# 7IBBE77S/nbodysim

Measured on AMD Instinct MI355X. Metric: particle-pair interactions/sec at N=262,144 (direct O(N^2) softened gravity + kick/drift step), higher is better.
Workload: dtype f32

## Files before the change

### include/nbody.h

```cpp
#ifndef NBODY_H
#define NBODY_H

#include <stddef.h>
#include <stdint.h>

#ifdef __cplusplus
extern "C" {
#endif
#pragma GCC visibility push(default)

#define NB_ABI_VERSION 8

typedef struct nb_vec2 {
    float x, y;
    float _pad[2];
} nb_vec2;

#define NB_Z(v) ((v)._pad[0])

typedef struct nb_body {
    nb_vec2 pos;
    nb_vec2 vel;
    nb_vec2 acc;
    float   mass;
// ... 69 lines not shown
       NB_INTEGRATOR_KDK = 1 };

enum { NB_FLAG_NO_SYMMETRY     = 1,
       NB_FLAG_NO_UNIFORM_MASS = 2,
       NB_FLAG_NO_GUIDED_TAIL  = 4,
       NB_FLAG_SHARD_ALLREDUCE = 8,
       NB_FLAG_MASS_SCALING    = 32,
       NB_FLAG_MASS_SCALING_MEASURED = 1024,
       NB_FLAG_NO_MASS_SCALING = 512,
       NB_FLAG_STATIC_ITEMS    = 256,
       NB_FLAG_SHARD_SINGLE    = 16,
       NB_FLAG_TREE_LEAVES     = 4096,
       NB_FLAG_TREE_QUADRUPOLE = 8192,
       NB_FLAG_TREE_ENERGY = 16384,
       NB_FLAG_TREE_RELATIVE = 32768 };
enum { NB_FLAGS_KNOWN = NB_FLAG_NO_SYMMETRY | NB_FLAG_NO_UNIFORM_MASS | NB_FLAG_NO_GUIDED_TAIL | NB_FLAG_SHARD_ALLREDUCE | NB_FLAG_SHARD_SINGLE |
                        NB_FLAG_MASS_SCALING | NB_FLAG_NO_MASS_SCALING | NB_FLAG_STATIC_ITEMS | NB_FLAG_MASS_SCALING_MEASURED |
                        NB_FLAG_TREE_LEAVES | NB_FLAG_TREE_QUADRUPOLE | NB_FLAG_TREE_ENERGY | NB_FLAG_TREE_RELATIVE };

typedef struct nb_params {
    uint32_t struct_size;
    float    eps;
    float    dt;
    int32_t  precision;
    int32_t  rsqrt_mode;
    int32_t  sum_order;
    int32_t  integrator;
    int32_t  extras;
    int32_t  device;
    int32_t  j_slices;
    uint64_t i_begin;
    uint64_t i_count;
    void    *stream;
// ... 63 lines not shown
    uint32_t struct_size;
    uint32_t width, height;
    float    center_x, center_y, scale;
    float    mass_quantum;
    uint32_t _reserved0;
} nb_view;
int nb_raster(nb_sim *s, const nb_view *view, uint32_t *count, float *mass);

#define NB_NO_NEIGHBOR 0xFFFFFFFFu
int nb_neighbors(nb_sim *s, float radius, uint32_t k, uint32_t *idx, float *dist2, uint32_t *count);

int nb_groups(nb_sim *s, float radius, uint32_t *label, uint32_t *size, uint64_t *ngroups);

int nb_tree_alpha(nb_sim *s, float alpha);

uint64_t nb_frame(const nb_sim *s);
size_t   nb_count(const nb_sim *s);
size_t   nb_owned_begin(const nb_sim *s);
size_t   nb_owned_count(const nb_sim *s);

int nb_dump(nb_sim *s, const char *path);
int nb_write_bodies(const char *path, const nb_body *bodies, size_t n, uint64_t frame,
                    const nb_params *params);
int nb_read_header(const char *path, size_t *n, uint64_t *frame, nb_params *params);
int nb_read_bodies(const char *path, nb_body *out, size_t n);

enum { NB_POS_CURRENT = 0, NB_POS_NEXT = 1 };
enum { NB_SHARD_NONE = 0, NB_SHARD_ALLGATHER = 1, NB_SHARD_SYMMETRIC = 2, NB_SHARD_ALLREDUCE = 3 };
int   nb_shard_protocol(const nb_sim *s);
int   nb_exchange_positions(nb_sim *const *sims, int count);
// ... 74 lines not shown
```

### nbodysim_amd/_lib.py

```python
from __future__ import annotations

import ctypes as C
import os
from pathlib import Path

import numpy as np

PKG_DIR = Path(__file__).resolve().parent
LIB_PATH = PKG_DIR / "libnbody_hip.so"

NB_ABI_VERSION = 8

NB_OK, NB_EINVAL, NB_ENODEVICE, NB_EHIP, NB_ENOMEM, NB_EIO, NB_EFORMAT, NB_ESTATE = 0, -1, -2, -3, -4, -5, -6, -7
NB_FP32, NB_FP64 = 0, 1
NB_RSQRT_EXACT, NB_RSQRT_QUAKE = 0, 1
NB_SUM_TILED, NB_SUM_SEQUENTIAL = 0, 1
NB_EXTRA_VCLAMP, NB_EXTRA_BOUNDARY, NB_EXTRA_COLLIDE = 1, 2, 4
NB_INTEGRATOR_KICK_DRIFT, NB_INTEGRATOR_KDK = 0, 1
NB_FORCE_DIRECT, NB_FORCE_TREE = 0, 1
NB_POS_CURRENT, NB_POS_NEXT = 0, 1
NB_SHARD_NONE, NB_SHARD_ALLGATHER, NB_SHARD_SYMMETRIC, NB_SHARD_ALLREDUCE = 0, 1, 2, 3
NB_FLAG_NO_SYMMETRY, NB_FLAG_NO_UNIFORM_MASS, NB_FLAG_NO_GUIDED_TAIL, NB_FLAG_SHARD_ALLREDUCE, NB_FLAG_SHARD_SINGLE, NB_FLAG_MASS_SCALING = 1, 2, 4, 8, 16, 32
NB_FLAG_STATIC_ITEMS = 256
NB_FLAG_NO_MASS_SCALING = 512
NB_FLAG_MASS_SCALING_MEASURED = 1024
NB_FLAG_TREE_LEAVES = 4096
NB_FLAG_TREE_QUADRUPOLE = 8192
NB_FLAG_TREE_ENERGY = 16384
NB_FLAG_TREE_RELATIVE = 32768
NB_NO_NEIGHBOR = 0xFFFFFFFF

BODY_DTYPE = np.dtype(
    {
        "names": ["pos", "vel", "acc", "mass", "radius"],
        "formats": [(np.float32, 2), (np.float32, 2), (np.float32, 2), np.float32, np.float32],
        "offsets": [0, 16, 32, 48, 52],
        "itemsize": 64,
    }
)


BODY3_DTYPE = np.dtype(
    {
        "names": ["pos", "vel", "acc", "mass", "radius"],
# ... 131 lines not shown
    "nb_snapshot_wait": (C.c_int, [C.c_void_p]),
    "nb_host_register": (C.c_int, [C.c_void_p, C.c_size_t]),
    "nb_host_unregister": (C.c_int, [C.c_void_p]),
    "nb_host_alloc": (C.c_void_p, [C.c_size_t]),
    "nb_host_free": (C.c_int, [C.c_void_p]),
    "nb_upload": (C.c_int, [C.c_void_p, C.c_void_p]),
    "nb_accelerations": (C.c_int, [C.c_void_p]),
    "nb_energy": (C.c_int, [C.c_void_p, C.POINTER(C.c_double), C.POINTER(C.c_double)]),
    "nb_momentum": (C.c_int, [C.c_void_p, C.POINTER(C.c_double), C.POINTER(C.c_double)]),
    "nb_potentials": (C.c_int, [C.c_void_p, C.c_void_p]),
    "nb_collide_capacity": (C.c_int, [C.c_void_p, C.c_size_t]),
    "nb_collision_stats": (C.c_int, [C.c_void_p, C.POINTER(C.c_uint64), C.POINTER(C.c_uint64), C.POINTER(C.c_uint32), C.POINTER(C.c_uint64)]),
    "nb_tree_stats": (C.c_int, [C.c_void_p, C.POINTER(C.c_uint64), C.POINTER(C.c_uint32), C.POINTER(C.c_uint64)]),
    "nb_tree_nodes": (C.c_int, [C.c_void_p, C.c_void_p, C.c_size_t, C.POINTER(C.c_size_t)]),
    "nb_tree_alpha": (C.c_int, [C.c_void_p, C.c_float]),
    "nb_raster": (C.c_int, [C.c_void_p, C.POINTER(nb_view), C.c_void_p, C.c_void_p]),
    "nb_neighbors": (C.c_int, [C.c_void_p, C.c_float, C.c_uint32, C.c_void_p, C.c_void_p, C.c_void_p]),
    "nb_groups": (C.c_int, [C.c_void_p, C.c_float, C.c_void_p, C.c_void_p, C.POINTER(C.c_uint64)]),
    "nb_frame": (C.c_uint64, [C.c_void_p]),
    "nb_count": (C.c_size_t, [C.c_void_p]),
    "nb_owned_begin": (C.c_size_t, [C.c_void_p]),
    "nb_owned_count": (C.c_size_t, [C.c_void_p]),
    "nb_dump": (C.c_int, [C.c_void_p, C.c_char_p]),
    "nb_write_bodies": (C.c_int, [C.c_char_p, C.c_void_p, C.c_size_t, C.c_uint64, C.POINTER(nb_params)]),
    "nb_read_header": (C.c_int, [C.c_char_p, C.POINTER(C.c_size_t), C.POINTER(C.c_uint64), C.POINTER(nb_params)]),
    "nb_read_bodies": (C.c_int, [C.c_char_p, C.c_void_p, C.c_size_t]),
    "nb_step_begin": (C.c_int, [C.c_void_p, C.c_float]),
    "nb_step_mid": (C.c_int, [C.c_void_p]),
    "nb_step_finish": (C.c_int, [C.c_void_p]),
    "nb_pos_buffer": (C.c_void_p, [C.c_void_p, C.c_int]),
# ... 129 lines not shown
```

### nbodysim_amd/csrc/nb_capi.hip

```cpp
#include "nb_sim.hip.h"

extern "C" int nb_device_count(void)
{
    int n = 0;
    if (hipGetDeviceCount(&n) != hipSuccess) { (void)hipGetLastError(); return 0; }
    return n;
}

static uint32_t even_slices(uint32_t jn, uint32_t want)
{
    const uint32_t tiles = (jn + TJ - 1) / TJ;
    if (want < 1) want = 1;
    if (want > tiles) want = tiles;
    const uint32_t per = (tiles + want - 1) / want;
    return (tiles + per - 1) / per;
}

static ForceJob plan_job(const nb_sim *s, uint32_t jb, uint32_t je, uint32_t slab0,
                         uint32_t gap_begin = 0xffffffffu, uint32_t gap_len = 0)
{
    ForceJob j{jb, je, 0, slab0, 1, 0, gap_begin, gap_len};
    const uint32_t ic = (uint32_t)s->i_count;
    if (je <= jb) return j;
    const uint32_t jn = je - jb;
// ... 28 lines not shown
    s->slabs_all = s->path == StepPath::SYM ? 1 : s->job_all.js;
    s->job_local = plan_job(s, ib, ib + ic, 0);
    s->job_remote = plan_job(s, 0, n - ic, s->job_local.js, ib, ic);
    s->slabs_two_phase = s->job_local.js + s->job_remote.js;
}

static bool needs_guard(const nb_sim *s) { return s->fp64 ? !(s->p.eps > 0.0f) : !(s->p.eps >= 1e-12f); }

static uint32_t sym_tile_of(const nb_params &p, size_t n)
{
    if (p.precision == NB_FP64 || p.dims == 3 || p.shard_world > 1 || (p.flags & NB_FLAG_SHARD_SINGLE)) return SYM_SB;
    if (p.sym_tile) return (uint32_t)p.sym_tile;
    return n < SYM_WS_MAX_N ? SYM_SB_WS : SYM_SB;
}

static bool sym_eligible(const nb_sim *s)
{
    if (s->p.flags & NB_FLAG_NO_SYMMETRY) return false;
    if (s->p.sum_order != NB_SUM_TILED || needs_guard(s)) return false;
    if (s->fp64 && s->p.rsqrt_mode != NB_RSQRT_EXACT) return false;
    if (s->p.integrator != NB_INTEGRATOR_KICK_DRIFT && s->i_count != s->n) return false;
    if (s->n < (sym_tile_of(s->p, s->n) == SYM_SB_WS ? (size_t)5632 : 8 * (size_t)SYM_SB)) return false;
    const uint32_t world = s->p.shard_world > 1 ? (uint32_t)s->p.shard_world : 1u;
    size_t cap = (size_t)96 << 30;
    if (world == 1) {
        size_t free_b = 0, total_b = 0;
        if (hipMemGetInfo(&free_b, &total_b) != hipSuccess) { (void)hipGetLastError(); free_b = (size_t)24 << 30; }
        if (free_b / 3 < cap) cap = free_b / 3;
    }
    if (sym_slab_r_bound((uint32_t)s->n, world, sym_tile_of(s->p, s->n)) * s->esz > cap) return false;
    return true;
}

static bool single_rank(const nb_sim *s)
{
    return (s->p.flags & NB_FLAG_SHARD_SINGLE) && s->p.shard_world == 1 && s->p.shard_rank == 0 && s->i_count == s->n;
}
// ... 352 lines not shown

static int query_stage(nb_sim *s, size_t bytes)
{
    HIPCHK(s->pool.regrow_pinned(s->qstage_cap, bytes, s->qstage));
    return NB_OK;
}

static int copy_plane(nb_sim *s, void *dst, const void *src, size_t bytes) { return copy_d2h(s, dst, src, bytes, s->stream, s->qstage); }

#include "nb_collide_host.hip.h"
#include "nb_tree_host.hip.h"
#include "nb_raster_host.hip.h"
#include "nb_potential_host.hip.h"
#include "nb_neighbors_host.hip.h"
#include "nb_groups_host.hip.h"

static int step_check(nb_sim *s)
{
    const int rc = collide_check(s);
    return rc ? rc : tree_check(s);
}

static int do_upload(nb_sim *s, const nb_body *in)
{
    { const int rc = fence_foreign_work(s); if (rc) return rc; }
    s->uniform_mass = s->n > 0 && !s->tree && !(s->p.flags & NB_FLAG_NO_UNIFORM_MASS) && s->p.sum_order == NB_SUM_TILED;
    for (size_t i = 1; s->uniform_mass && i < s->n; ++i)
        if (memcmp(&in[i].mass, &in[0].mass, sizeof(float)) != 0) s->uniform_mass = false;
    s->um_mass = in[0].mass;
    s->mass_scaled = false;
// ... 20 lines not shown
    const uint32_t n = (uint32_t)s->n, g = (n + BLOCK - 1) / BLOCK, ib = (uint32_t)s->i_begin, ic = (uint32_t)s->i_count;
    with_layout(s, [&](auto L) {
        using real = typename decltype(L)::real;
        using vec = typename decltype(L)::vec;
        for (int b = 0; b < 2; ++b)
            unpack_bodies<decltype(L)><<<g, BLOCK, 0, s->stream>>>(s->aos_dev, n, (vec *)s->pos[b], (real *)s->mass, (vec *)s->vel, (vec *)s->acc,
                                                                   s->radius, ib, ic);
    });
    HIPCHK(hipGetLastError());
    if (forced_scaling || auto_scaling) {
        if (!s->sigma) HIPCHK(s->pool.alloc(s->sigma, s->n));
        mass_sigma<<<g, BLOCK, 0, s->stream>>>((const float *)s->mass, s->sigma, n);
        HIPCHK(hipGetLastError());
    }
    s->mass_scaled = forced_scaling;
    if (s->collide) { const int rc = collide_classify(s, in); if (rc) return rc; }
    HIPCHK(hipStreamSynchronize(s->stream));
    s->acc_valid = false;
    if (auto_scaling) { const int rc = choose_mass_scaling(s); if (rc) return rc; }
    if (auto_scaling || was_uniform != s->uniform_mass || was_scaled != s->mass_scaled) s->sym_first_wave = 0;
    s->sym_first_wave_uniform = s->uniform_mass;
    s->sym_first_wave_scaled = s->mass_scaled;
    return NB_OK;
}

extern "C" nb_sim *nb_create(const nb_body *init, size_t n, const nb_params *params)
{
    nb_clear_error();
    nb_params p;
    if (params) {
// ... 131 lines not shown
    s->bh.theta2 = p.theta * p.theta;
    s->bh.leaves = s->tree && (p.flags & NB_FLAG_TREE_LEAVES) != 0;
    s->bh.quad = s->bh.leaves && (p.flags & NB_FLAG_TREE_QUADRUPOLE) != 0;
    s->bh.energy = s->bh.leaves && (p.flags & NB_FLAG_TREE_ENERGY) != 0;
    s->bh.rel = s->bh.leaves && (p.flags & NB_FLAG_TREE_RELATIVE) != 0;
    if ((e = s->pool.alloc(s->mass, n * s->rsz)) != hipSuccess) return fail("allocating mass", e);
    if ((e = s->pool.alloc(s->radius, n)) != hipSuccess) return fail("allocating radius", e);
    if ((e = s->pool.alloc(s->vel, s->i_count * r2)) != hipSuccess) return fail("allocating vel", e);
    if ((e = s->pool.alloc(s->acc, s->i_count * r2)) != hipSuccess) return fail("allocating acc", e);
    if ((e = s->pool.alloc(s->partial, s->tree ? r2 : (size_t)s->slabs_cap * s->i_count * r2)) != hipSuccess) return fail("allocating partial", e);
    if ((e = s->pool.alloc(s->aos_dev, n)) != hipSuccess) return fail("allocating aos", e);
    s->ered_blocks = (s->i_count + BLOCK - 1) / BLOCK;
    if ((e = s->pool.alloc(s->ered_dev, (s->bh.energy ? 4 : 2) * s->ered_blocks)) != hipSuccess) return fail("allocating energy", e);

    s->collide = (p.extras & NB_EXTRA_COLLIDE) != 0;
    if ((symmetric(s) && plan_sym(s) != NB_OK) || (s->collide && collide_alloc(s) != NB_OK) || (s->tree && tree_alloc(s) != NB_OK) ||
        do_upload(s, init) != NB_OK) { free_all(s); (void)hipGetLastError(); return nullptr; }
    return s;
}

extern "C" void nb_destroy(nb_sim *s) { free_all(s); }

extern "C" int nb_upload(nb_sim *s, const nb_body *in)
{
    if (!s || !in) return nb_fail(NB_EINVAL, "nb_upload: NULL argument");
    if (bind(s)) return NB_EHIP;
    if (snapshot_wait(s)) return nb_last_error_code();
    return do_upload(s, in);
}

static int prof_begin(nb_sim *s, std::pair<hipEvent_t, hipEvent_t> *pr, hipStream_t st)
{
// ... 60 lines not shown

static int launch_sym_items(nb_sim *s, uint32_t first, uint32_t count, hipStream_t st = nullptr)
{
    if (count == 0) return NB_OK;
    if (!st) st = s->stream;
    std::pair<hipEvent_t, hipEvent_t> pr;
    if (s->prof && prof_begin(s, &pr, st)) return NB_EHIP;
    const uint32_t n = (uint32_t)s->n;
    const SymItem *items = s->sym_items_dev + first;
    const uint32_t slot = first == 0 ? 0u : (first == s->sym_items_local ? 1u : 2u);
    const bool quake = s->p.rsqrt_mode == NB_RSQRT_QUAKE, um = s->uniform_mass, pairs = sym_uses_pairs(s);
    const int rc = with_layout(s, [&](auto L) -> int {
        using real = typename decltype(L)::real;
        using vec = typename decltype(L)::vec;
        const real eps2 = (real)s->p.eps * (real)s->p.eps, umv = um ? (real)s->um_mass : (real)1;
        const vec *pos = (const vec *)s->pos[s->cur];
        vec *ss = (vec *)s->sym_slab_s, *sr = (vec *)s->sym_slab_r;
        auto go = [&](auto kernel, auto... lead) { return launch_sym_kernel(s, kernel, count, slot, st, lead..., items, ss, sr, n, eps2, umv); };
        if constexpr (L.dims3 && std::is_same_v<real, double>)
            return with_flags([&](auto u) { return go(force_sym3_f64<u>, pos); }, um);
        else if constexpr (L.dims3)
            return with_flags([&](auto q, auto u, auto pp) { return go(force_sym3_f32<q ? RSQ_QUAKE : RSQ_EXACT, u, pp>, pos); }, quake, um, pairs);
        else if constexpr (std::is_same_v<real, double>)
            return with_flags([&](auto u) { return go(force_sym_f64<u>, pos, (const double *)s->mass); }, um);
        else
            return with_flags([&](auto q, auto pp, auto ws) {
                constexpr int RQ = q ? RSQ_QUAKE : RSQ_EXACT;
                const float *mass = (const float *)s->mass;
                if (um) return go(force_sym_f32<RQ, MM_UNIFORM, pp, ws>, pos, mass, s->sigma);
                if constexpr (RQ == RSQ_EXACT && !pp)
                    if (s->mass_scaled) return go(force_sym_f32<RSQ_EXACT, MM_SCALED, false, ws>, pos, mass, s->sigma);
                return go(force_sym_f32<RQ, MM_GENERAL, pp, ws>, pos, mass, s->sigma);
            }, quake, pairs, s->sym_sb == SYM_SB_WS);
    });
    if (rc) return rc;
    if (s->prof && prof_end(s, pr, st)) return NB_EHIP;
    return NB_OK;
}

static int launch_gather(nb_sim *s, bool fuse, const uint32_t *lo, const uint32_t *hi, const uint32_t *cb, const SymCov *cov,
                         uint32_t first, uint32_t cnt, void *dst, const void *add, double dt)
{
    const uint32_t n = (uint32_t)s->n, per = s->dims3 ? (uint32_t)GATHER_T : (uint32_t)GATHER_P, gg = (cnt + per - 1) / per;
    const int extras = fuse ? s->p.extras : 0, kd = fuse ? INTEG_KICK | INTEG_DRIFT : 0;
    with_layout(s, [&](auto L) {
        using real = typename decltype(L)::real;
        using vec = typename decltype(L)::vec;
        const vec *ss = (const vec *)s->sym_slab_s, *sr = (const vec *)s->sym_slab_r;
        const vec *pc = fuse ? (const vec *)s->pos[s->cur] : nullptr;
        vec *pn = fuse ? (vec *)s->pos[s->cur ^ 1] : nullptr, *vel = fuse ? (vec *)s->vel : nullptr, *acc = fuse ? (vec *)s->acc : nullptr;
        const real h = fuse ? (real)dt : (real)0;
        with_flags([&](auto f) {
            if constexpr (L.dims3)
                sym_gather3<real, f><<<gg, BLOCK, 0, s->stream>>>(ss, sr, lo, hi, cb, cov, n, first, cnt, (vec *)dst, (const vec *)add,
                                                                  pc, pn, vel, acc, h, h, kd);
            else
                sym_gather<real, f><<<gg, BLOCK, 0, s->stream>>>(ss, sr, lo, hi, cb, cov, n, first, cnt, (vec *)dst, (const vec *)add,
                                                                 pc, pn, vel, acc, h, h, extras, kd, s->sym_sb_shift);
        }, fuse);
    });
    HIPCHK(hipGetLastError());
    return NB_OK;
}

static int launch_sym_gather(nb_sim *s, bool fuse_step, double dt)
{
    void *dst = s->path == StepPath::SYM ? s->partial : s->acc_full;
    return launch_gather(s, fuse_step, s->sym_rowbase_dev, s->sym_rowbase_dev + s->sym_tiles,
                         s->sym_cov_begin_dev, s->sym_cov_dev, 0u, (uint32_t)s->n, dst, nullptr, dt);
}

static int launch_sym_gather_late(nb_sim *s, double dt)
{
    const uint32_t tiles = s->sym_tiles;
    return launch_gather(s, true, s->sym_rowbase_dev + tiles, s->sym_rowbase_dev + 2 * (size_t)tiles,
                         s->sym_cov_begin_dev + (tiles + 1), s->sym_cov_dev + s->sym_cov_late_off,
                         (uint32_t)s->i_begin, (uint32_t)s->i_count, nullptr, s->acc_owned, dt);
}

static int launch_force_sym(nb_sim *s, bool fuse_step = false, double dt = 0.0)
{
    int rc = launch_sym_items(s, 0, s->sym_items);
    if (rc) return rc;
    return launch_sym_gather(s, fuse_step, dt);
}

static int launch_force(nb_sim *s, const ForceJob &j)
{
    if (j.j_end <= j.j_begin || j.js == 0) return NB_OK;
    if (s->tree) return nb_fail(NB_ESTATE, "internal: a direct-sum force launch on a NB_FORCE_TREE handle (it has no partial slabs)");
    if (s->path == StepPath::SYM && &j == &s->job_all) return launch_force_sym(s);
    std::pair<hipEvent_t, hipEvent_t> pr;
    if (s->prof && prof_begin(s, &pr)) return NB_EHIP;
    const bool guard = needs_guard(s), quake = s->p.rsqrt_mode == NB_RSQRT_QUAKE;
    const bool um = s->uniform_mass && !guard, scaled = s->mass_scaled && !guard;
    const uint32_t ib = (uint32_t)s->i_begin, ic = (uint32_t)s->i_count, grid = grid_blocks(j.i_tiles, j.js);
    with_layout(s, [&](auto L) {
        using Lt = decltype(L);
// ... 668 lines not shown
    if (symmetric(s)) *out = s->sym_info;
    else { memset(out, 0, sizeof *out); out->struct_size = (uint32_t)sizeof(nb_sym_info); out->cus = (uint32_t)s->cus; }
    return NB_OK;
}

extern "C" int nb_describe(nb_sim *s, char *buf, size_t buflen)
{
    if (!s || !buf || !buflen) return nb_fail(NB_EINVAL, "nb_describe: NULL argument");
    const ForceJob &a = s->job_all;
    const bool seq = s->p.sum_order == NB_SUM_SEQUENTIAL;
    const char *resolve = "none";
    if (s->collide) {
        if (bind(s) || collide_read(s)) return nb_last_error_code();
        resolve = s->coll.host->touched == 0 ? "none" : s->coll.host->lds_last ? "lds" : "global";
    }
    const int used = snprintf(buf, buflen,
             "n=%zu owned=[%zu,+%zu) %s%s rsqrt=%s sum=%s | force: block=%d waves/i-set=%d i/lane=%d i_tiles=%u j_slices(all)=%u grid=%u tile_j=%d | "
             "two-phase P/slices local=%d/%u remote=%d/%u | uniform_mass=%d mass_scaled=%d mass_scaling_check=%.1e | symmetric=%d tile=%u chunk_pairs=%d items=%u chunks/item=%u late=%u slabs=%.1f+%.1f MiB | CUs=%d",
             s->n, s->i_begin, s->i_count, s->fp64 ? "fp64" : "fp32", s->dims3 ? " 3-D" : "",
             s->p.rsqrt_mode == NB_RSQRT_QUAKE ? "quake" : "exact", seq ? "sequential" : "tiled",
             BLOCK, (seq || s->fp64) ? 1 : TILED_F32_WS, seq ? 1 : (s->fp64 ? a.P : 2 * a.P), a.i_tiles, a.js,
             seq ? a.i_tiles : grid_blocks(a.i_tiles, a.js), TJ,
             s->job_local.P, s->job_local.js, s->job_remote.P, s->job_remote.js, (int)s->uniform_mass, (int)s->mass_scaled, (double)s->mass_scaling_dev,
             (int)symmetric(s), s->sym_sb, (int)sym_uses_pairs(s), s->sym_items, s->sym_L, s->sym_items_late,
             (double)s->sym_info.slab_s_bytes / 1048576.0, (double)s->sym_info.slab_r_bytes / 1048576.0, s->cus);
    if (used >= 0 && (size_t)used < buflen)
        snprintf(buf + used, buflen - (size_t)used, " | collide=%d h=%.6g large=%u capacity=%llu resolve=%s", (int)s->collide, s->coll.h,
                 s->coll.large_n, (unsigned long long)s->coll.cap, resolve);
    const size_t len = strlen(buf);
    if (len < buflen) {
        if (s->tree) snprintf(buf + len, buflen - len, " | force=tree theta=%.6g node_capacity=%llu depth_cap=%d%s%s%s", (double)s->p.theta,
                              (unsigned long long)s->bh.cap, TREE_DEPTH_CAP,
                              !s->bh.leaves ? "" : tree_walk_is_group(s) ? " leaves=1 walk=group" : " leaves=1 walk=lane",
                              s->bh.quad ? " quad=1" : "", s->bh.energy ? " energy=tree" : "");
        else snprintf(buf + len, buflen - len, " | force=direct");
        const size_t len2 = strlen(buf);
        if (s->bh.rel && len2 < buflen) snprintf(buf + len2, buflen - len2, " alpha=%.6g", (double)s->bh.alpha);
    }
    return NB_OK;
}
// ... 1 lines not shown
```

### nbodysim_amd/csrc/nb_kernels.hip.h

```cpp
#pragma once
#include <hip/hip_runtime.h>
#include <stdint.h>
#include <type_traits>

#include "nb_plan.h"

namespace nbk {

typedef float v2f __attribute__((ext_vector_type(2)));
typedef float v4f __attribute__((ext_vector_type(4)));

constexpr int BLOCK = 256;
constexpr int TJ = 256;

enum { RSQ_EXACT = 0, RSQ_QUAKE = 1 };

constexpr float PAD_XY = 1.0e18f;

template <typename real> struct vec2_of;
template <> struct vec2_of<float> { typedef float2 type; };
template <> struct vec2_of<double> { typedef double2 type; };

template <typename real> struct vec4_of;
template <> struct vec4_of<float> { typedef float4 type; };
// ... 764 lines not shown
        mu = mu > m2 ? mu : m2;
    }
    if ((threadIdx.x & 63u) == 0u) { atomicMax(&out[0], du); atomicMax(&out[1], mu); }
}

constexpr int GATHER_Q = 8, GATHER_T = BLOCK / GATHER_Q, GATHER_V = 2, GATHER_P = GATHER_T * GATHER_V;
static_assert(SYM_SB % GATHER_P == 0 && SYM_SB_WS % GATHER_P == 0, "the particles of a gather workgroup share a tile");

__device__ __forceinline__ void load_pair(const float2 *__restrict__ p, float2 &a, float2 &b)
{
    const float4 v = *reinterpret_cast<const float4 *>(p);
    a = make_float2(v.x, v.y); b = make_float2(v.z, v.w);
}
__device__ __forceinline__ void load_pair(const double2 *__restrict__ p, double2 &a, double2 &b) { a = p[0]; b = p[1]; }

template <typename real, bool FUSE>
__device__ __forceinline__
void sym_gather_block(uint32_t blk,
                const typename vec2_of<real>::type *__restrict__ slab_s,
                const typename vec2_of<real>::type *__restrict__ slab_r,
                const uint32_t *__restrict__ row_lo, const uint32_t *__restrict__ row_hi,
                const uint32_t *__restrict__ cov_begin, const SymCov *__restrict__ cov,
                uint32_t n, uint32_t k0, uint32_t kn,
                typename vec2_of<real>::type *__restrict__ acc_sum,
                const typename vec2_of<real>::type *__restrict__ base,
                const typename vec2_of<real>::type *__restrict__ pos_cur,
                typename vec2_of<real>::type *__restrict__ pos_next,
                typename vec2_of<real>::type *__restrict__ vel,
                typename vec2_of<real>::type *__restrict__ acc,
                real dt_kick, real dt_drift, int extras, int flags, uint32_t sb_shift)
{
    typedef typename vec2_of<real>::type real2;
    __shared__ real2 part[GATHER_Q][GATHER_P];
    const uint32_t p = threadIdx.x % GATHER_T, q = threadIdx.x / GATHER_T;
    const uint32_t li = blk * GATHER_P + 2u * p, k = k0 + li;
    real2 a0, a1; a0.x = a0.y = a1.x = a1.y = 0;
    const uint32_t f = threadIdx.x, lf = blk * GATHER_P + f;
    real2 vf, xf; vf.x = vf.y = xf.x = xf.y = 0;
    if constexpr (FUSE) { if (f < (uint32_t)GATHER_P && lf < kn && (flags & INTEG_KICK)) { vf = vel[lf]; xf = pos_cur[k0 + lf]; } }
    if (li < kn) {
        const uint32_t g = k >> sb_shift, loc = k & ((1u << sb_shift) - 1u);
        const uint32_t r0 = row_lo[g], r1 = row_hi[g];
#pragma unroll 4
        for (uint32_t r = r0 + q; r < r1; r += GATHER_Q) {
            real2 b0, b1;
            load_pair(slab_s + ((size_t)r << sb_shift) + loc, b0, b1);
            a0.x += b0.x; a0.y += b0.y; a1.x += b1.x; a1.y += b1.y;
        }
        const uint32_t c1 = cov_begin[g + 1];
        for (uint32_t i = cov_begin[g] + q; i < c1; i += 4u * GATHER_Q) {
            SymCov cv[4];
            bool in[4];
#pragma unroll
            for (int u = 0; u < 4; ++u) {
// ... 11 lines not shown
            for (int u = 0; u < 4; ++u) {
                if (!in[u]) continue;
                a0.x += b0[u].x; a0.y += b0[u].y;
                if (k + 1 < cv[u].hi) { a1.x += b1[u].x; a1.y += b1[u].y; }
            }
        }
    }
    part[q][2u * p] = a0;
    part[q][2u * p + 1] = a1;
    __syncthreads();
    if (f < (uint32_t)GATHER_P && lf < kn) {
        real2 t = part[0][f];
#pragma unroll
        for (int j = 1; j < GATHER_Q; ++j) { t.x += part[j][f].x; t.y += part[j][f].y; }
        if (base) { const real2 bb = base[lf]; t.x += bb.x; t.y += bb.y; }
        if constexpr (FUSE) kick_drift_loaded<Layout<real, false>, false>(t, vf, xf, lf, pos_next, vel, acc, k0, dt_kick, dt_drift, extras, flags);
        else acc_sum[k0 + lf] = t;
    }
}

template <typename real, bool FUSE>
__global__ __launch_bounds__(BLOCK)
void sym_gather(const typename vec2_of<real>::type *__restrict__ slab_s,
                const typename vec2_of<real>::type *__restrict__ slab_r,
                const uint32_t *__restrict__ row_lo, const uint32_t *__restrict__ row_hi,
                const uint32_t *__restrict__ cov_begin, const SymCov *__restrict__ cov,
                uint32_t n, uint32_t k0, uint32_t kn,
                typename vec2_of<real>::type *__restrict__ acc_sum,
                const typename vec2_of<real>::type *__restrict__ base,
                const typename vec2_of<real>::type *__restrict__ pos_cur,
                typename vec2_of<real>::type *__restrict__ pos_next,
                typename vec2_of<real>::type *__restrict__ vel,
                typename vec2_of<real>::type *__restrict__ acc,
                real dt_kick, real dt_drift, int extras, int flags, uint32_t sb_shift)
{
    sym_gather_block<real, FUSE>(blockIdx.x, slab_s, slab_r, row_lo, row_hi, cov_begin, cov, n, k0, kn, acc_sum, base, pos_cur, pos_next, vel, acc,
                                 dt_kick, dt_drift, extras, flags, sb_shift);
}

constexpr int SYM_P64 = 8;
__device__ __forceinline__ double vgpr_const(double k);
__device__ __forceinline__ double rsqrt_f64(double x, double k0375);
__device__ __forceinline__ double rsqrt3_f64(double x, double k15, double k1875);

__device__ __forceinline__ double lane_rot64(double v, int addr)
{
    const unsigned long long u = __builtin_bit_cast(unsigned long long, v);
    const unsigned lo = (unsigned)__builtin_amdgcn_ds_bpermute(addr, (int)(unsigned)u);
    const unsigned hi = (unsigned)__builtin_amdgcn_ds_bpermute(addr, (int)(unsigned)(u >> 32));
    return __builtin_bit_cast(double, ((unsigned long long)hi << 32) | lo);
}

// ... 466 lines not shown
```

### nbodysim_amd/csrc/nb_sim.hip.h

```cpp
#pragma once
#include "nbody.h"
#include "nbody_debug.h"
#include "nb_internal.h"
#include "nb_kernels.hip.h"
#include "nb_kernels3d.hip.h"
#include "nb_collide.hip.h"
#include "nb_tree.hip.h"
#include "nb_raster.hip.h"
#include "nb_potential.hip.h"
#include "nb_neighbors.hip.h"
#include "nb_groups.hip.h"

#include <hip/hip_runtime.h>

#include <algorithm>
#include <cmath>
#include <cstdarg>
#include <cstdio>
#include <cstdlib>
#include <cstring>
#include <mutex>
#include <new>
#include <type_traits>
#include <vector>

#include <unistd.h>
// ... 188 lines not shown
        uint32_t *cnt = nullptr;
        uint64_t idx_cap = 0, d2_cap = 0;
        uint32_t *idx = nullptr;
        float *d2 = nullptr;
    } nbr;

    struct Groups {
        uint64_t cap = 0;
        uint32_t *parent = nullptr;
        uint32_t *cnt = nullptr;
        uint32_t *size = nullptr;
        uint32_t *words = nullptr;
        uint32_t *host = nullptr;
    } grp;

    bool prof = false;
    std::vector<std::pair<hipEvent_t, hipEvent_t>> ev_pool, ev_used;
    std::vector<uint32_t> ev_weight;
    double prof_ms = 0.0;
    uint64_t prof_launches = 0;
};

static int bind(const nb_sim *s)
{
    int d = -1;
    HIPCHK(hipGetDevice(&d));
    if (d != s->dev) HIPCHK(hipSetDevice(s->dev));
    return NB_OK;
}

// ... 30 lines not shown
```

### nbodysim_amd/simulation.py

```python
from __future__ import annotations

import ctypes as C
from typing import Optional

import numpy as np

from . import _lib as L

SIMULATION_DT: float = 0.01


class Simulation:

    def __init__(
        self,
        bodies: np.ndarray,
        eps: float = 1.0,
        precision: str = "fp32",
        rsqrt: str = "exact",
        order: str = "tiled",
        integrator: str = "kick_drift",
        extras: int = 0,
        device: int = -1,
        j_slices: int = 0,
# ... 17 lines not shown
        first_frame: int = 0,
        shard_single: bool = False,
        mass_scaling=False,
        sym_chunk_pairs: int = 0,
        sym_tile: int = 0,
        pos_rows: int = 0,
        static_items: bool = False,
        collide: bool = False,
        force: str = "direct",
        theta: float = 1.0,
        library=None,
        tree_leaves: bool = False,
        tree_quadrupole: bool = False,
        tree_energy: bool = False,
        tree_alpha: Optional[float] = None,
    ):
        if tree_leaves and force != "tree":
            raise ValueError('tree_leaves=True needs force="tree" (NB_FLAG_TREE_LEAVES selects a walk of the Barnes-Hut force)')
        if tree_quadrupole and not (force == "tree" and tree_leaves):
            raise ValueError('tree_quadrupole=True needs force="tree" and tree_leaves=True (NB_FLAG_TREE_QUADRUPOLE adds a term to the '
                             "accepted cells of the convergent Barnes-Hut force)")
        if tree_energy and not (force == "tree" and tree_leaves):
            raise ValueError('tree_energy=True needs force="tree" and tree_leaves=True (NB_FLAG_TREE_ENERGY makes energy() walk the tree '
                             "of the convergent Barnes-Hut force)")
        if tree_alpha is not None and not (force == "tree" and tree_leaves):
            raise ValueError('tree_alpha needs force="tree" and tree_leaves=True (NB_FLAG_TREE_RELATIVE adds an acceleration-relative '
                             "opening test to the walks of the convergent Barnes-Hut force)")
        lib = library if library is not None else L.load()
        if bodies.dtype not in (L.BODY_DTYPE, L.BODY3_DTYPE):
            raise TypeError("bodies must be a numpy array of nbodysim_amd.BODY_DTYPE (64-byte Body records)")
# ... 13 lines not shown
        p.j_slices = j_slices
        p.i_begin = i_begin
        p.i_count = i_count
        if stream is not None:
            p.stream = stream
        if pos_buffers is not None:
            p.pos_buffers[0], p.pos_buffers[1] = pos_buffers
        p.dims = dims
        p.flags = ((0 if symmetry else L.NB_FLAG_NO_SYMMETRY) | (0 if uniform_mass else L.NB_FLAG_NO_UNIFORM_MASS)
                   | (0 if guided_tail else L.NB_FLAG_NO_GUIDED_TAIL) | (L.NB_FLAG_SHARD_ALLREDUCE if shard_allreduce else 0)
                   | (L.NB_FLAG_SHARD_SINGLE if shard_single else 0)
                   | (L.NB_FLAG_MASS_SCALING_MEASURED if mass_scaling == "measured" else L.NB_FLAG_MASS_SCALING if mass_scaling is True
                      else L.NB_FLAG_NO_MASS_SCALING if mass_scaling is False else 0)
                   | (L.NB_FLAG_STATIC_ITEMS if static_items else 0) | (L.NB_FLAG_TREE_LEAVES if tree_leaves else 0)
                   | (L.NB_FLAG_TREE_QUADRUPOLE if tree_quadrupole else 0) | (L.NB_FLAG_TREE_ENERGY if tree_energy else 0)
                   | (L.NB_FLAG_TREE_RELATIVE if tree_alpha is not None else 0))
        p.sym_chunks_per_item, p.sym_aux_stream, p.sym_late_us, p.lanes_p = sym_chunks_per_item, sym_aux_stream, sym_late_us, lanes_p
        if sym_tail is not None:
            p.sym_tail[0], p.sym_tail[1], p.sym_tail[2] = sym_tail
        p.first_frame = first_frame
        p.sym_chunk_pairs = sym_chunk_pairs
        p.sym_tile = sym_tile
        p.pos_rows = pos_rows
        p.force = {"direct": L.NB_FORCE_DIRECT, "tree": L.NB_FORCE_TREE}[force]
        p.theta = theta
        p.shard_rank, p.shard_world = shard_rank, shard_world
        if acc_buffers is not None:
            p.acc_buffers[0], p.acc_buffers[1] = acc_buffers
        self._lib = lib
        self._params = p
        self._h = lib.nb_create(bodies.ctypes.data, bodies.shape[0], C.byref(p))
# ... 149 lines not shown
        out = tuple(a for a in (idx, d2, cnt) if a is not None)
        return out[0] if len(out) == 1 else out

    def groups(self, radius: float, size: bool = False, ngroups: bool = False):
        label = np.empty(self.i_count, dtype=np.uint32)
        sizes = np.empty(self.i_count, dtype=np.uint32) if size else None
        count = C.c_uint64(0)
        L.check("nb_groups", self._lib.nb_groups(self._h, radius, label.ctypes.data, sizes.ctypes.data if size else None,
                                                 C.byref(count) if ngroups else None), self._lib)
        out = (label,) + ((sizes,) if size else ()) + ((int(count.value),) if ngroups else ())
        return out[0] if len(out) == 1 else out

    def set_tree_alpha(self, alpha: float) -> None:
        L.check("nb_tree_alpha", self._lib.nb_tree_alpha(self._h, alpha), self._lib)

    def dump(self, path: str) -> None:
        L.check("nb_dump", self._lib.nb_dump(self._h, str(path).encode()), self._lib)

    def step_begin(self, dt: Optional[float] = None) -> None:
        L.check("nb_step_begin", self._lib.nb_step_begin(self._h, SIMULATION_DT if dt is None else dt), self._lib)

    def step_mid(self) -> None:
        L.check("nb_step_mid", self._lib.nb_step_mid(self._h), self._lib)

    def step_finish(self) -> None:
        L.check("nb_step_finish", self._lib.nb_step_finish(self._h), self._lib)

    def pos_buffer(self, which: int = L.NB_POS_CURRENT) -> int:
        return int(self._lib.nb_pos_buffer(self._h, which) or 0)

# ... 63 lines not shown
```

Measured before the change: 9539 billion.

## Sweep symmetric direct-force pairs over Morton-ordered body copies

```diff
diff --git a/include/nbody.h b/include/nbody.h
--- a/include/nbody.h
+++ b/include/nbody.h
@@ -107,9 +107,12 @@
        NB_FLAG_TREE_QUADRUPOLE = 8192,
        NB_FLAG_TREE_ENERGY = 16384,
        NB_FLAG_TREE_RELATIVE = 32768 };
+enum { NB_FLAG_BODY_ORDER    = 131072,
+       NB_FLAG_NO_BODY_ORDER = 262144 };
 enum { NB_FLAGS_KNOWN = NB_FLAG_NO_SYMMETRY | NB_FLAG_NO_UNIFORM_MASS | NB_FLAG_NO_GUIDED_TAIL | NB_FLAG_SHARD_ALLREDUCE | NB_FLAG_SHARD_SINGLE |
                         NB_FLAG_MASS_SCALING | NB_FLAG_NO_MASS_SCALING | NB_FLAG_STATIC_ITEMS | NB_FLAG_MASS_SCALING_MEASURED |
-                        NB_FLAG_TREE_LEAVES | NB_FLAG_TREE_QUADRUPOLE | NB_FLAG_TREE_ENERGY | NB_FLAG_TREE_RELATIVE };
+                        NB_FLAG_TREE_LEAVES | NB_FLAG_TREE_QUADRUPOLE | NB_FLAG_TREE_ENERGY | NB_FLAG_TREE_RELATIVE |
+                        NB_FLAG_BODY_ORDER | NB_FLAG_NO_BODY_ORDER };
 
 typedef struct nb_params {
     uint32_t struct_size;
@@ -203,6 +206,8 @@
 
 int nb_tree_alpha(nb_sim *s, float alpha);
 
+int nb_body_order(nb_sim *s, uint32_t every, uint32_t *perm_out, uint32_t *every_out);
+
 uint64_t nb_frame(const nb_sim *s);
 size_t   nb_count(const nb_sim *s);
 size_t   nb_owned_begin(const nb_sim *s);
diff --git a/nbodysim_amd/_lib.py b/nbodysim_amd/_lib.py
--- a/nbodysim_amd/_lib.py
+++ b/nbodysim_amd/_lib.py
@@ -28,6 +28,8 @@
 NB_FLAG_TREE_QUADRUPOLE = 8192
 NB_FLAG_TREE_ENERGY = 16384
 NB_FLAG_TREE_RELATIVE = 32768
+NB_FLAG_BODY_ORDER = 131072
+NB_FLAG_NO_BODY_ORDER = 262144
 NB_NO_NEIGHBOR = 0xFFFFFFFF
 
 BODY_DTYPE = np.dtype(
@@ -189,6 +191,7 @@
     "nb_tree_stats": (C.c_int, [C.c_void_p, C.POINTER(C.c_uint64), C.POINTER(C.c_uint32), C.POINTER(C.c_uint64)]),
     "nb_tree_nodes": (C.c_int, [C.c_void_p, C.c_void_p, C.c_size_t, C.POINTER(C.c_size_t)]),
     "nb_tree_alpha": (C.c_int, [C.c_void_p, C.c_float]),
+    "nb_body_order": (C.c_int, [C.c_void_p, C.c_uint32, C.c_void_p, C.POINTER(C.c_uint32)]),
     "nb_raster": (C.c_int, [C.c_void_p, C.POINTER(nb_view), C.c_void_p, C.c_void_p]),
     "nb_neighbors": (C.c_int, [C.c_void_p, C.c_float, C.c_uint32, C.c_void_p, C.c_void_p, C.c_void_p]),
     "nb_groups": (C.c_int, [C.c_void_p, C.c_float, C.c_void_p, C.c_void_p, C.POINTER(C.c_uint64)]),
diff --git a/nbodysim_amd/csrc/nb_capi.hip b/nbodysim_amd/csrc/nb_capi.hip
--- a/nbodysim_amd/csrc/nb_capi.hip
+++ b/nbodysim_amd/csrc/nb_capi.hip
@@ -66,13 +66,31 @@
     return n < SYM_WS_MAX_N ? SYM_SB_WS : SYM_SB;
 }
 
+constexpr size_t ORDER_MIN_N = 131072, ORDER_MAX_N = 262144;
+
+static bool order_possible(const nb_params &p, size_t n, size_t i_count)
+{
+    return !(p.flags & NB_FLAG_NO_BODY_ORDER) && p.force == NB_FORCE_DIRECT && p.dims != 3 && p.shard_world <= 1 &&
+           !(p.flags & NB_FLAG_SHARD_SINGLE) && i_count == n;
+}
+
+static bool order_forced(const nb_sim *s) { return (s->p.flags & NB_FLAG_BODY_ORDER) && order_possible(s->p, s->n, s->i_count); }
+
+static bool order_wanted(const nb_sim *s)
+{
+    if (s->path != StepPath::SYM || !order_possible(s->p, s->n, s->i_count)) return false;
+    if (s->p.flags & NB_FLAG_BODY_ORDER) return true;
+    const bool scaling = (s->p.flags & (NB_FLAG_MASS_SCALING | NB_FLAG_MASS_SCALING_MEASURED)) && !(s->p.flags & NB_FLAG_NO_MASS_SCALING);
+    return s->n >= ORDER_MIN_N && s->n <= ORDER_MAX_N && !scaling;
+}
+
 static bool sym_eligible(const nb_sim *s)
 {
     if (s->p.flags & NB_FLAG_NO_SYMMETRY) return false;
     if (s->p.sum_order != NB_SUM_TILED || needs_guard(s)) return false;
     if (s->fp64 && s->p.rsqrt_mode != NB_RSQRT_EXACT) return false;
     if (s->p.integrator != NB_INTEGRATOR_KICK_DRIFT && s->i_count != s->n) return false;
-    if (s->n < (sym_tile_of(s->p, s->n) == SYM_SB_WS ? (size_t)5632 : 8 * (size_t)SYM_SB)) return false;
+    if (!order_forced(s) && s->n < (sym_tile_of(s->p, s->n) == SYM_SB_WS ? (size_t)5632 : 8 * (size_t)SYM_SB)) return false;
     const uint32_t world = s->p.shard_world > 1 ? (uint32_t)s->p.shard_world : 1u;
     size_t cap = (size_t)96 << 30;
     if (world == 1) {
@@ -455,6 +473,7 @@
 #include "nb_potential_host.hip.h"
 #include "nb_neighbors_host.hip.h"
 #include "nb_groups_host.hip.h"
+#include "nb_order_host.hip.h"
 
 static int step_check(nb_sim *s)
 {
@@ -505,6 +524,7 @@
         HIPCHK(hipGetLastError());
     }
     s->mass_scaled = forced_scaling;
+    if (s->ord.on) { const int rc = order_upload(s); if (rc) return rc; }
     if (s->collide) { const int rc = collide_classify(s, in); if (rc) return rc; }
     HIPCHK(hipStreamSynchronize(s->stream));
     s->acc_valid = false;
@@ -666,8 +686,9 @@
     if ((e = s->pool.alloc(s->ered_dev, (s->bh.energy ? 4 : 2) * s->ered_blocks)) != hipSuccess) return fail("allocating energy", e);
 
     s->collide = (p.extras & NB_EXTRA_COLLIDE) != 0;
-    if ((symmetric(s) && plan_sym(s) != NB_OK) || (s->collide && collide_alloc(s) != NB_OK) || (s->tree && tree_alloc(s) != NB_OK) ||
-        do_upload(s, init) != NB_OK) { free_all(s); (void)hipGetLastError(); return nullptr; }
+    s->ord.on = order_wanted(s);
+    if ((symmetric(s) && plan_sym(s) != NB_OK) || (s->ord.on && order_alloc(s) != NB_OK) || (s->collide && collide_alloc(s) != NB_OK) ||
+        (s->tree && tree_alloc(s) != NB_OK) || do_upload(s, init) != NB_OK) { free_all(s); (void)hipGetLastError(); return nullptr; }
     return s;
 }
 
@@ -758,7 +779,7 @@
         using real = typename decltype(L)::real;
         using vec = typename decltype(L)::vec;
         const real eps2 = (real)s->p.eps * (real)s->p.eps, umv = um ? (real)s->um_mass : (real)1;
-        const vec *pos = (const vec *)s->pos[s->cur];
+        const vec *pos = (const vec *)sym_positions(s);
         vec *ss = (vec *)s->sym_slab_s, *sr = (vec *)s->sym_slab_r;
         auto go = [&](auto kernel, auto... lead) { return launch_sym_kernel(s, kernel, count, slot, st, lead..., items, ss, sr, n, eps2, umv); };
         if constexpr (L.dims3 && std::is_same_v<real, double>)
@@ -766,15 +787,15 @@
         else if constexpr (L.dims3)
             return with_flags([&](auto q, auto u, auto pp) { return go(force_sym3_f32<q ? RSQ_QUAKE : RSQ_EXACT, u, pp>, pos); }, quake, um, pairs);
         else if constexpr (std::is_same_v<real, double>)
-            return with_flags([&](auto u) { return go(force_sym_f64<u>, pos, (const double *)s->mass); }, um);
+            return with_flags([&](auto u) { return go(force_sym_f64<u>, pos, (const double *)sym_masses(s)); }, um);
         else
             return with_flags([&](auto q, auto pp, auto ws) {
                 constexpr int RQ = q ? RSQ_QUAKE : RSQ_EXACT;
-                const float *mass = (const float *)s->mass;
-                if (um) return go(force_sym_f32<RQ, MM_UNIFORM, pp, ws>, pos, mass, s->sigma);
+                const float *mass = (const float *)sym_masses(s), *sigma = sym_sigma(s);
+                if (um) return go(force_sym_f32<RQ, MM_UNIFORM, pp, ws>, pos, mass, sigma);
                 if constexpr (RQ == RSQ_EXACT && !pp)
-                    if (s->mass_scaled) return go(force_sym_f32<RSQ_EXACT, MM_SCALED, false, ws>, pos, mass, s->sigma);
-                return go(force_sym_f32<RQ, MM_GENERAL, pp, ws>, pos, mass, s->sigma);
+                    if (s->mass_scaled) return go(force_sym_f32<RSQ_EXACT, MM_SCALED, false, ws>, pos, mass, sigma);
+                return go(force_sym_f32<RQ, MM_GENERAL, pp, ws>, pos, mass, sigma);
             }, quake, pairs, s->sym_sb == SYM_SB_WS);
     });
     if (rc) return rc;
@@ -799,8 +820,10 @@
                 sym_gather3<real, f><<<gg, BLOCK, 0, s->stream>>>(ss, sr, lo, hi, cb, cov, n, first, cnt, (vec *)dst, (const vec *)add,
                                                                   pc, pn, vel, acc, h, h, kd);
             else
-                sym_gather<real, f><<<gg, BLOCK, 0, s->stream>>>(ss, sr, lo, hi, cb, cov, n, first, cnt, (vec *)dst, (const vec *)add,
-                                                                 pc, pn, vel, acc, h, h, extras, kd, s->sym_sb_shift);
+                with_flags([&](auto o) {
+                    sym_gather<real, f, o><<<gg, BLOCK, 0, s->stream>>>(ss, sr, lo, hi, cb, cov, n, first, cnt, (vec *)dst, (const vec *)add,
+                                                                        pc, pn, vel, acc, h, h, extras, kd, s->sym_sb_shift, o ? s->ord.perm : nullptr);
+                }, s->ord.on);
         }, fuse);
     });
     HIPCHK(hipGetLastError());
@@ -824,8 +847,9 @@
 
 static int launch_force_sym(nb_sim *s, bool fuse_step = false, double dt = 0.0)
 {
-    int rc = launch_sym_items(s, 0, s->sym_items);
-    if (rc) return rc;
+    int rc;
+    if (s->ord.on && (rc = order_prepare(s))) return rc;
+    if ((rc = launch_sym_items(s, 0, s->sym_items))) return rc;
     return launch_sym_gather(s, fuse_step, dt);
 }
 
@@ -1524,7 +1548,7 @@
         if (bind(s) || collide_read(s)) return nb_last_error_code();
         resolve = s->coll.host->touched == 0 ? "none" : s->coll.host->lds_last ? "lds" : "global";
     }
-    const int used = snprintf(buf, buflen,
+    int used = snprintf(buf, buflen,
              "n=%zu owned=[%zu,+%zu) %s%s rsqrt=%s sum=%s | force: block=%d waves/i-set=%d i/lane=%d i_tiles=%u j_slices(all)=%u grid=%u tile_j=%d | "
              "two-phase P/slices local=%d/%u remote=%d/%u | uniform_mass=%d mass_scaled=%d mass_scaling_check=%.1e | symmetric=%d tile=%u chunk_pairs=%d items=%u chunks/item=%u late=%u slabs=%.1f+%.1f MiB | CUs=%d",
              s->n, s->i_begin, s->i_count, s->fp64 ? "fp64" : "fp32", s->dims3 ? " 3-D" : "",
@@ -1534,6 +1558,10 @@
              s->job_local.P, s->job_local.js, s->job_remote.P, s->job_remote.js, (int)s->uniform_mass, (int)s->mass_scaled, (double)s->mass_scaling_dev,
              (int)symmetric(s), s->sym_sb, (int)sym_uses_pairs(s), s->sym_items, s->sym_L, s->sym_items_late,
              (double)s->sym_info.slab_s_bytes / 1048576.0, (double)s->sym_info.slab_r_bytes / 1048576.0, s->cus);
+    if (used >= 0 && (size_t)used < buflen) {
+        if (s->ord.on) used += snprintf(buf + used, buflen - (size_t)used, " order=morton/%u", s->ord.every);
+        else used += snprintf(buf + used, buflen - (size_t)used, " order=0");
+    }
     if (used >= 0 && (size_t)used < buflen)
         snprintf(buf + used, buflen - (size_t)used, " | collide=%d h=%.6g large=%u capacity=%llu resolve=%s", (int)s->collide, s->coll.h,
                  s->coll.large_n, (unsigned long long)s->coll.cap, resolve);
diff --git a/nbodysim_amd/csrc/nb_kernels.hip.h b/nbodysim_amd/csrc/nb_kernels.hip.h
--- a/nbodysim_amd/csrc/nb_kernels.hip.h
+++ b/nbodysim_amd/csrc/nb_kernels.hip.h
@@ -802,7 +802,7 @@
 }
 __device__ __forceinline__ void load_pair(const double2 *__restrict__ p, double2 &a, double2 &b) { a = p[0]; b = p[1]; }
 
-template <typename real, bool FUSE>
+template <typename real, bool FUSE, bool ORD = false>
 __device__ __forceinline__
 void sym_gather_block(uint32_t blk,
                 const typename vec2_of<real>::type *__restrict__ slab_s,
@@ -816,7 +816,7 @@
                 typename vec2_of<real>::type *__restrict__ pos_next,
                 typename vec2_of<real>::type *__restrict__ vel,
                 typename vec2_of<real>::type *__restrict__ acc,
-                real dt_kick, real dt_drift, int extras, int flags, uint32_t sb_shift)
+                real dt_kick, real dt_drift, int extras, int flags, uint32_t sb_shift, const uint32_t *__restrict__ perm = nullptr)
 {
     typedef typename vec2_of<real>::type real2;
     __shared__ real2 part[GATHER_Q][GATHER_P];
@@ -825,7 +825,9 @@
     real2 a0, a1; a0.x = a0.y = a1.x = a1.y = 0;
     const uint32_t f = threadIdx.x, lf = blk * GATHER_P + f;
     real2 vf, xf; vf.x = vf.y = xf.x = xf.y = 0;
-    if constexpr (FUSE) { if (f < (uint32_t)GATHER_P && lf < kn && (flags & INTEG_KICK)) { vf = vel[lf]; xf = pos_cur[k0 + lf]; } }
+    uint32_t of = lf;
+    if constexpr (ORD) { if (f < (uint32_t)GATHER_P && lf < kn) of = perm[lf]; }
+    if constexpr (FUSE) { if (f < (uint32_t)GATHER_P && lf < kn && (flags & INTEG_KICK)) { vf = vel[of]; xf = pos_cur[k0 + of]; } }
     if (li < kn) {
         const uint32_t g = k >> sb_shift, loc = k & ((1u << sb_shift) - 1u);
         const uint32_t r0 = row_lo[g], r1 = row_hi[g];
@@ -867,12 +869,12 @@
 #pragma unroll
         for (int j = 1; j < GATHER_Q; ++j) { t.x += part[j][f].x; t.y += part[j][f].y; }
         if (base) { const real2 bb = base[lf]; t.x += bb.x; t.y += bb.y; }
-        if constexpr (FUSE) kick_drift_loaded<Layout<real, false>, false>(t, vf, xf, lf, pos_next, vel, acc, k0, dt_kick, dt_drift, extras, flags);
-        else acc_sum[k0 + lf] = t;
-    }
-}
-
-template <typename real, bool FUSE>
+        if constexpr (FUSE) kick_drift_loaded<Layout<real, false>, false>(t, vf, xf, of, pos_next, vel, acc, k0, dt_kick, dt_drift, extras, flags);
+        else acc_sum[k0 + of] = t;
+    }
+}
+
+template <typename real, bool FUSE, bool ORD = false>
 __global__ __launch_bounds__(BLOCK)
 void sym_gather(const typename vec2_of<real>::type *__restrict__ slab_s,
                 const typename vec2_of<real>::type *__restrict__ slab_r,
@@ -885,10 +887,10 @@
                 typename vec2_of<real>::type *__restrict__ pos_next,
                 typename vec2_of<real>::type *__restrict__ vel,
                 typename vec2_of<real>::type *__restrict__ acc,
-                real dt_kick, real dt_drift, int extras, int flags, uint32_t sb_shift)
-{
-    sym_gather_block<real, FUSE>(blockIdx.x, slab_s, slab_r, row_lo, row_hi, cov_begin, cov, n, k0, kn, acc_sum, base, pos_cur, pos_next, vel, acc,
-                                 dt_kick, dt_drift, extras, flags, sb_shift);
+                real dt_kick, real dt_drift, int extras, int flags, uint32_t sb_shift, const uint32_t *__restrict__ perm)
+{
+    sym_gather_block<real, FUSE, ORD>(blockIdx.x, slab_s, slab_r, row_lo, row_hi, cov_begin, cov, n, k0, kn, acc_sum, base, pos_cur, pos_next, vel, acc,
+                                      dt_kick, dt_drift, extras, flags, sb_shift, perm);
 }
 
 constexpr int SYM_P64 = 8;
diff --git a/nbodysim_amd/csrc/nb_order.hip.h b/nbodysim_amd/csrc/nb_order.hip.h
--- /dev/null
+++ b/nbodysim_amd/csrc/nb_order.hip.h
@@ -0,0 +1,89 @@
+#pragma once
+#include "nb_kernels.hip.h"
+
+#ifndef NB_ORDER_EVERY
+#define NB_ORDER_EVERY 16
+#endif
+
+namespace nbk {
+
+constexpr uint32_t ORDER_PARTS = 256;
+
+__device__ __forceinline__ float order_div(float a, float b) { return __fdiv_rn(a, b); }
+__device__ __forceinline__ double order_div(double a, double b) { return __ddiv_rn(a, b); }
+
+template <typename real>
+__device__ __forceinline__ void order_block_box(real &lx, real &ly, real &hx, real &hy)
+{
+    __shared__ real sh[4][BLOCK];
+    const uint32_t t = threadIdx.x;
+    sh[0][t] = lx; sh[1][t] = ly; sh[2][t] = hx; sh[3][t] = hy;
+    __syncthreads();
+    for (uint32_t s = BLOCK / 2; s > 0; s >>= 1) {
+        if (t < s) {
+            sh[0][t] = fmin(sh[0][t], sh[0][t + s]); sh[1][t] = fmin(sh[1][t], sh[1][t + s]);
+            sh[2][t] = fmax(sh[2][t], sh[2][t + s]); sh[3][t] = fmax(sh[3][t], sh[3][t + s]);
+        }
+        __syncthreads();
+    }
+    lx = sh[0][0]; ly = sh[1][0]; hx = sh[2][0]; hy = sh[3][0];
+    __syncthreads();
+}
+
+template <typename real>
+__global__ __launch_bounds__(BLOCK)
+void order_bounds(const typename vec2_of<real>::type *__restrict__ pos, uint32_t n, real *__restrict__ part)
+{
+    real lx = INFINITY, ly = INFINITY, hx = -INFINITY, hy = -INFINITY;
+    for (uint32_t i = blockIdx.x * BLOCK + threadIdx.x; i < n; i += gridDim.x * BLOCK) {
+        const auto p = pos[i];
+        lx = fmin(lx, p.x); ly = fmin(ly, p.y); hx = fmax(hx, p.x); hy = fmax(hy, p.y);
+    }
+    order_block_box(lx, ly, hx, hy);
+    if (threadIdx.x == 0) { part[4u * blockIdx.x] = lx; part[4u * blockIdx.x + 1] = ly; part[4u * blockIdx.x + 2] = hx; part[4u * blockIdx.x + 3] = hy; }
+}
+
+__device__ __forceinline__ uint32_t order_spread(uint32_t v)
+{
+    v = (v | (v << 8)) & 0x00FF00FFu;
+    v = (v | (v << 4)) & 0x0F0F0F0Fu;
+    v = (v | (v << 2)) & 0x33333333u;
+    v = (v | (v << 1)) & 0x55555555u;
+    return v;
+}
+
+template <typename real>
+__device__ __forceinline__ uint32_t order_axis(real x, real lo, real hi)
+{
+    if (!(hi > lo)) return 0u;
+    const real t = order_div(x - lo, hi - lo) * (real)65536;
+    if (!(t >= (real)0)) return 0u;
+    return t >= (real)65535 ? 65535u : (uint32_t)t;
+}
+
+template <typename real>
+__global__ __launch_bounds__(BLOCK)
+void order_keys(const typename vec2_of<real>::type *__restrict__ pos, uint32_t n, const real *__restrict__ part, uint32_t nparts,
+                uint64_t *__restrict__ key, uint32_t *__restrict__ val)
+{
+    static_assert(ORDER_PARTS <= (uint32_t)BLOCK, "one partial box per thread");
+    real lx = INFINITY, ly = INFINITY, hx = -INFINITY, hy = -INFINITY;
+    if (threadIdx.x < nparts) { lx = part[4u * threadIdx.x]; ly = part[4u * threadIdx.x + 1]; hx = part[4u * threadIdx.x + 2]; hy = part[4u * threadIdx.x + 3]; }
+    order_block_box(lx, ly, hx, hy);
+    const uint32_t i = blockIdx.x * BLOCK + threadIdx.x;
+    if (i >= n) return;
+    const auto p = pos[i];
+    const uint32_t m = order_spread(order_axis(p.x, lx, hx)) | (order_spread(order_axis(p.y, ly, hy)) << 1);
+    key[i] = ((uint64_t)m << 32) | i;
+    val[i] = i;
+}
+
+template <typename T>
+__global__ __launch_bounds__(BLOCK)
+void order_permute(const T *__restrict__ src, const uint32_t *__restrict__ perm, uint32_t n, T *__restrict__ dst)
+{
+    const uint32_t k = blockIdx.x * BLOCK + threadIdx.x;
+    if (k < n) dst[k] = src[perm[k]];
+}
+
+}
diff --git a/nbodysim_amd/csrc/nb_order_host.hip.h b/nbodysim_amd/csrc/nb_order_host.hip.h
--- /dev/null
+++ b/nbodysim_amd/csrc/nb_order_host.hip.h
@@ -0,0 +1,86 @@
+#pragma once
+
+static int order_alloc(nb_sim *s)
+{
+    nb_sim::Order &o = s->ord;
+    const size_t n = s->n;
+    HIPCHK(s->pool.alloc(o.perm, n));
+    HIPCHK(s->pool.alloc(o.val, n));
+    HIPCHK(s->pool.alloc(o.key, n));
+    HIPCHK(s->pool.alloc(o.skey, n));
+    HIPCHK(s->pool.alloc(o.part, (size_t)ORDER_PARTS * 4 * s->rsz));
+    HIPCHK(s->pool.alloc(o.xs, n * s->esz));
+    size_t bytes = 0;
+    HIPCHK(nb_tree_sort_pairs(nullptr, bytes, o.key, o.skey, o.val, o.perm, n, s->stream));
+    o.tmp_bytes = std::max<size_t>(bytes, 256);
+    HIPCHK(s->pool.alloc(o.tmp, o.tmp_bytes));
+    return NB_OK;
+}
+
+static int order_upload(nb_sim *s)
+{
+    nb_sim::Order &o = s->ord;
+    if (!s->uniform_mass && !o.ms) HIPCHK(s->pool.alloc(o.ms, s->n * s->rsz));
+    if (s->sigma && !o.sigma_s) HIPCHK(s->pool.alloc(o.sigma_s, s->n));
+    o.evals = 0;
+    return NB_OK;
+}
+
+static int order_sort(nb_sim *s)
+{
+    nb_sim::Order &o = s->ord;
+    const uint32_t n = (uint32_t)s->n, g = (n + BLOCK - 1) / BLOCK, parts = g < ORDER_PARTS ? g : ORDER_PARTS;
+    with_layout(s, [&](auto L) {
+        using real = typename decltype(L)::real;
+        if constexpr (!L.dims3) {
+            using vec = typename decltype(L)::vec;
+            const vec *pos = (const vec *)s->pos[s->cur];
+            order_bounds<real><<<parts, BLOCK, 0, s->stream>>>(pos, n, (real *)o.part);
+            order_keys<real><<<g, BLOCK, 0, s->stream>>>(pos, n, (const real *)o.part, parts, o.key, o.val);
+        }
+    });
+    HIPCHK(hipGetLastError());
+    size_t tmp = o.tmp_bytes;
+    HIPCHK(nb_tree_sort_pairs(o.tmp, tmp, o.key, o.skey, o.val, o.perm, n, s->stream));
+    if (!s->uniform_mass) {
+        if (s->fp64) order_permute<double><<<g, BLOCK, 0, s->stream>>>((const double *)s->mass, o.perm, n, (double *)o.ms);
+        else order_permute<float><<<g, BLOCK, 0, s->stream>>>((const float *)s->mass, o.perm, n, (float *)o.ms);
+    }
+    if (s->sigma) order_permute<float><<<g, BLOCK, 0, s->stream>>>(s->sigma, o.perm, n, o.sigma_s);
+    HIPCHK(hipGetLastError());
+    return NB_OK;
+}
+
+static int order_prepare(nb_sim *s)
+{
+    nb_sim::Order &o = s->ord;
+    if (o.evals % o.every == 0) { const int rc = order_sort(s); if (rc) return rc; }
+    ++o.evals;
+    const uint32_t n = (uint32_t)s->n, g = (n + BLOCK - 1) / BLOCK;
+    if (s->fp64) order_permute<double2><<<g, BLOCK, 0, s->stream>>>((const double2 *)s->pos[s->cur], o.perm, n, (double2 *)o.xs);
+    else order_permute<float2><<<g, BLOCK, 0, s->stream>>>((const float2 *)s->pos[s->cur], o.perm, n, (float2 *)o.xs);
+    HIPCHK(hipGetLastError());
+    return NB_OK;
+}
+
+static const void *sym_positions(const nb_sim *s) { return s->ord.on ? s->ord.xs : s->pos[s->cur]; }
+static const void *sym_masses(const nb_sim *s) { return s->ord.on && !s->uniform_mass ? s->ord.ms : s->mass; }
+static const float *sym_sigma(const nb_sim *s) { return s->ord.on && s->sigma ? s->ord.sigma_s : s->sigma; }
+
+extern "C" int nb_body_order(nb_sim *s, uint32_t every, uint32_t *perm_out, uint32_t *every_out)
+{
+    if (!s) return nb_fail(NB_EINVAL, "nb_body_order: NULL handle");
+    if (!s->ord.on) {
+        if (every_out) *every_out = 0u;
+        if (every || perm_out) return nb_fail(NB_ESTATE, "nb_body_order: the handle sweeps its bodies in the caller's order (nb_describe: order=0)");
+        return NB_OK;
+    }
+    if (every) s->ord.every = every;
+    if (every_out) *every_out = s->ord.every;
+    if (!perm_out) return NB_OK;
+    { const int rc = query_enter(s, "nb_body_order"); if (rc) return rc; }
+    if (s->ord.evals == 0) { const int rc = order_sort(s); if (rc) return rc; }
+    const size_t bytes = s->n * sizeof(uint32_t);
+    { const int rc = query_stage(s, stage_need(perm_out, bytes)); if (rc) return rc; }
+    return copy_plane(s, perm_out, s->ord.perm, bytes);
+}
diff --git a/nbodysim_amd/csrc/nb_sim.hip.h b/nbodysim_amd/csrc/nb_sim.hip.h
--- a/nbodysim_amd/csrc/nb_sim.hip.h
+++ b/nbodysim_amd/csrc/nb_sim.hip.h
@@ -10,6 +10,7 @@
 #include "nb_potential.hip.h"
 #include "nb_neighbors.hip.h"
 #include "nb_groups.hip.h"
+#include "nb_order.hip.h"
 
 #include <hip/hip_runtime.h>
 
@@ -228,6 +229,19 @@
         uint32_t *host = nullptr;
     } grp;
 
+    struct Order {
+        bool on = false;
+        uint32_t every = NB_ORDER_EVERY;
+        uint64_t evals = 0;
+        uint32_t *perm = nullptr, *val = nullptr;
+        uint64_t *key = nullptr, *skey = nullptr;
+        void *part = nullptr;
+        void *xs = nullptr, *ms = nullptr;
+        float *sigma_s = nullptr;
+        void *tmp = nullptr;
+        size_t tmp_bytes = 0;
+    } ord;
+
     bool prof = false;
     std::vector<std::pair<hipEvent_t, hipEvent_t>> ev_pool, ev_used;
     std::vector<uint32_t> ev_weight;
diff --git a/nbodysim_amd/simulation.py b/nbodysim_amd/simulation.py
--- a/nbodysim_amd/simulation.py
+++ b/nbodysim_amd/simulation.py
@@ -55,6 +55,7 @@
         tree_quadrupole: bool = False,
         tree_energy: bool = False,
         tree_alpha: Optional[float] = None,
+        body_order: Optional[bool] = None,
     ):
         if tree_leaves and force != "tree":
             raise ValueError('tree_leaves=True needs force="tree" (NB_FLAG_TREE_LEAVES selects a walk of the Barnes-Hut force)')
@@ -98,7 +99,8 @@
                       else L.NB_FLAG_NO_MASS_SCALING if mass_scaling is False else 0)
                    | (L.NB_FLAG_STATIC_ITEMS if static_items else 0) | (L.NB_FLAG_TREE_LEAVES if tree_leaves else 0)
                    | (L.NB_FLAG_TREE_QUADRUPOLE if tree_quadrupole else 0) | (L.NB_FLAG_TREE_ENERGY if tree_energy else 0)
-                   | (L.NB_FLAG_TREE_RELATIVE if tree_alpha is not None else 0))
+                   | (L.NB_FLAG_TREE_RELATIVE if tree_alpha is not None else 0)
+                   | (L.NB_FLAG_BODY_ORDER if body_order is True else L.NB_FLAG_NO_BODY_ORDER if body_order is False else 0))
         p.sym_chunks_per_item, p.sym_aux_stream, p.sym_late_us, p.lanes_p = sym_chunks_per_item, sym_aux_stream, sym_late_us, lanes_p
         if sym_tail is not None:
             p.sym_tail[0], p.sym_tail[1], p.sym_tail[2] = sym_tail
@@ -278,6 +280,12 @@
     def set_tree_alpha(self, alpha: float) -> None:
         L.check("nb_tree_alpha", self._lib.nb_tree_alpha(self._h, alpha), self._lib)
 
+    def body_order(self, every: int = 0, perm: bool = False):
+        out = np.empty(self.n, dtype=np.uint32) if perm else None
+        ev = C.c_uint32(0)
+        L.check("nb_body_order", self._lib.nb_body_order(self._h, every, out.ctypes.data if perm else None, C.byref(ev)), self._lib)
+        return (int(ev.value), out) if perm else int(ev.value)
+
     def dump(self, path: str) -> None:
         L.check("nb_dump", self._lib.nb_dump(self._h, str(path).encode()), self._lib)
 
```

Result: faster. 9895 billion, median of 6 (+3.7%).
